# pollen-robotics/reachy2_symbolic_ik

Hardware: NVIDIA B200
Metric: ik_poses_per_sec (higher is better)
Workload: dtype f64

## Files before the change

### reachy2_symbolic_ik_b200/csrc/r2ik_device.cuh

```cuda
#pragma once

#include <math.h>
#include <stdint.h>

#include "../../include/r2ik.h"
#include "r2ik_math.cuh"

namespace r2ik {

constexpr double kPi = 3.14159265358979323846;
constexpr double kTwoPi = 2.0 * kPi;
constexpr double kHalfPi = kPi / 2;

struct ArmConst {
  double s[3];
  double L1, L2, L12;
  double L1sq, L2sq;
  double wo[3];
  double to[3];
  double tip_z;
  double max_arm_length;
  double d_min;
  double proj_margin;
  double backward_limit;
  double nvm;
  double rL, rLsq, hL;
  double Mst[9];
  double Pst[3];
  double es[3];
  double sing_coeff, sing_offset;
  double plP[3], plV[3];
  double plC[3], plRho;
  double elbow_limit;
  double side;
};



template <bool LIT>
R2IK_HD void cs_of_atan2(double y, double x, double &c, double &s, bool &degenerate) {
  if (LIT) {
    sincos(atan2(y, x), &s, &c);
  } else {
    double h2 = x * x + y * y;
    degenerate = degenerate || !((unsigned)(hi_word(h2) - 0x05e00000) < (unsigned)(0x7a000000 - 0x05e00000));
    double ih = rsqrt_pos(h2);
    c = x * ih; s = y * ih;
  }
}

template <bool LIT>
R2IK_HD double cs_and_angle(double y, double x, double &c, double &s, bool &degenerate) {
  cs_of_atan2<LIT>(y, x, c, s, degenerate);
  if (LIT) return atan2(y, x);
  return angle_of_unit(c, s);
}

template <bool LIT>
R2IK_HD double atan2_leaf(double y, double x, bool &degenerate) {
  if (LIT) return atan2(y, x);
  degenerate = degenerate || !atan2_core_ok(y, x);
  return atan2_core(y, x);
}

#if defined(__CUDACC__)
__device__ __noinline__ double2 sincos_library_dev(double a) {
  double s, c;
  sincos(a, &s, &c);
  return make_double2(s, c);
}
#endif
R2IK_HD void sincos_any(double a, double &s, double &c) {
  if (sincos_small_ok(a)) { sincos_small(a, s, c); return; }
#if defined(__CUDA_ARCH__)
  double2 r = sincos_library_dev(a);
  s = r.x; c = r.y;
#else
  sincos(a, &s, &c);
#endif
}

R2IK_HD double pymod(double a, double m) {
  double r = fmod(a, m);
  if (r != 0.0) {
    if ((m < 0.0) != (r < 0.0)) r += m;
  } else {
    r = copysign(0.0, m);
  }
  return r;
}

R2IK_HD double pymod_2pi_not_minus_zero(double x) {
  const double two_pi = R2IK_WRAP(1), four_pi = R2IK_WRAP(2);
  if (!(x >= -two_pi && x < R2IK_WRAP(3))) return pymod(x, kTwoPi);
  double r = x >= four_pi ? x - four_pi : x;
  r = r >= two_pi ? r - two_pi : r;
  return x < 0.0 ? x + two_pi : r;
}
R2IK_HD double pymod_2pi(double x) { return pymod_2pi_not_minus_zero(x) + 0.0; }

R2IK_HD double angle_diff(double a, double b) { return pymod_2pi_not_minus_zero((a - b) + R2IK_WRAP(0)) - R2IK_WRAP(0); }

R2IK_HD bool np_isclose(double a, double b) { return fabs(a - b) <= 1e-8 + 1e-5 * fabs(b); }

R2IK_HD bool is_valid_angle(double angle, double i0, double i1) {
  if (pymod_2pi(i0) == pymod_2pi(i1)) return true;
  if (i0 < i1) return (i0 <= angle) && (angle <= i1);
  return (i0 <= angle) || (angle <= i1);
}

R2IK_HD double limit_theta_to_interval(double theta, double i0, double i1) {
  theta = pymod_2pi(theta);
  if (theta > kPi) theta -= kTwoPi;
  if (is_valid_angle(theta, i0, i1)) return theta;
  double pos_diff = angle_diff(theta, i1);
  double neg_diff = angle_diff(theta, i0);
  if (fabs(pos_diff) < fabs(neg_diff)) return i1;
  return i0;
}

R2IK_HD double mul_add_unfused(double a, double b, double c) {
#if defined(__CUDA_ARCH__)
  return __dadd_rn(__dmul_rn(a, b), c);
#else
  return a * b + c;
#endif
}

struct Linspace {
  double start, stop, delta, step;
  int div;
};
R2IK_HD Linspace make_linspace(double start, double stop, int num) {
  Linspace L;
  L.start = start; L.stop = stop; L.div = num - 1; L.delta = stop - start;
  L.step = L.div > 0 ? L.delta / (double)L.div : 0.0;
  return L;
}
R2IK_HD double linspace_value(const Linspace &L, int i) {
  if (L.div <= 0) return L.start;
  if (i == L.div) return L.stop;
  if (L.step == 0.0) return mul_add_unfused((double)i / (double)L.div, L.delta, L.start);
  return mul_add_unfused((double)i, L.step, L.start);
}

R2IK_HD void search_range(double i0, double i1, double &start, double &stop) {
  if (fabs(fabs(i0) + fabs(i1) - kTwoPi) < 0.00001) { start = kHalfPi; stop = kHalfPi + kTwoPi; }
  else if (i0 < i1) { start = i0; stop = i1; }
  else { start = i0; stop = i1 + kTwoPi; }
}

struct Quat { double x, y, z, w; };

R2IK_HD Quat quat_mul(const Quat &p, const Quat &q) {
  Quat o;
  o.x = p.w * q.x + q.w * p.x + (p.y * q.z - p.z * q.y);
  o.y = p.w * q.y + q.w * p.y + (p.z * q.x - p.x * q.z);
  o.z = p.w * q.z + q.w * p.z + (p.x * q.y - p.y * q.x);
  o.w = p.w * q.w - p.x * q.x - p.y * q.y - p.z * q.z;
  return o;
}

R2IK_HD Quat quat_axis(int axis, double angle) {
  double s, c;
  sincos(angle / 2.0, &s, &c);
  Quat q = {0.0, 0.0, 0.0, c};
  if (axis == 0) q.x = s; else if (axis == 1) q.y = s; else q.z = s;
  return q;
}

R2IK_HD Quat quat_from_euler(int a0, int a1, int a2, bool intrinsic, double e0, double e1, double e2) {
  Quat q = quat_axis(a0, e0);
  Quat q1 = quat_axis(a1, e1);
  q = intrinsic ? quat_mul(q, q1) : quat_mul(q1, q);
  Quat q2 = quat_axis(a2, e2);
  q = intrinsic ? quat_mul(q, q2) : quat_mul(q2, q);
  return q;
}

R2IK_HD void quat_to_matrix(const Quat &q, double m[9]) {
  double x2 = q.x * q.x, y2 = q.y * q.y, z2 = q.z * q.z, w2 = q.w * q.w;
  double xy = q.x * q.y, zw = q.z * q.w, xz = q.x * q.z, yw = q.y * q.w, yz = q.y * q.z, xw = q.x * q.w;
  m[0] = x2 - y2 - z2 + w2; m[1] = 2 * (xy - zw);       m[2] = 2 * (xz + yw);
  m[3] = 2 * (xy + zw);     m[4] = -x2 + y2 - z2 + w2;  m[5] = 2 * (yz - xw);
  m[6] = 2 * (xz - yw);     m[7] = 2 * (yz + xw);       m[8] = -x2 - y2 + z2 + w2;
}

R2IK_HD void rot_from_euler_xyz(double e0, double e1, double e2, double m[9]) {
  double sx, cx, sy, cy, sz, cz;
  sincos_any(e0 / 2.0, sx, cx);
  sincos_any(e1 / 2.0, sy, cy);
  sincos_any(e2 / 2.0, sz, cz);
  Quat a = {cy * sx, cx * sy, -(sy * sx), cy * cx};
  Quat q;
  q.x = cz * a.x - sz * a.y;
  q.y = cz * a.y + sz * a.x;
  q.z = cz * a.z + a.w * sz;
  q.w = cz * a.w - sz * a.z;
  quat_to_matrix(q, m);
}

R2IK_HD double det3(const double m[9]) {
  return m[0] * (m[4] * m[8] - m[5] * m[7]) - m[1] * (m[3] * m[8] - m[5] * m[6]) + m[2] * (m[3] * m[7] - m[4] * m[6]);
}

R2IK_HD void polar_orthogonalize(double m[9]) {
  double mx = 0.0;
  for (int k = 0; k < 9; ++k) mx = fmax(mx, fabs(m[k]));
  if (mx < 0.0625 || (mx > 16.0 && mx < INFINITY)) {
    const int e = ilogb(mx);
    for (int k = 0; k < 9; ++k) m[k] = ldexp(m[k], -e);
  }
  bool last = false;
  for (int it = 0; it < 60; ++it) {
    double id = 1.0 / det3(m);
    double c[9];
    c[0] = (m[4] * m[8] - m[5] * m[7]) * id; c[1] = (m[5] * m[6] - m[3] * m[8]) * id; c[2] = (m[3] * m[7] - m[4] * m[6]) * id;
    c[3] = (m[2] * m[7] - m[1] * m[8]) * id; c[4] = (m[0] * m[8] - m[2] * m[6]) * id; c[5] = (m[1] * m[6] - m[0] * m[7]) * id;
    c[6] = (m[1] * m[5] - m[2] * m[4]) * id; c[7] = (m[2] * m[3] - m[0] * m[5]) * id; c[8] = (m[0] * m[4] - m[1] * m[3]) * id;
    double delta = 0.0;
    for (int k = 0; k < 9; ++k) {
      double nx = 0.5 * (m[k] + c[k]);
      delta = fmax(delta, fabs(nx - m[k]));
      m[k] = nx;
    }
    if (last) break;
    if (delta < 1e-8) last = true;
  }
}

R2IK_HD bool quat_from_matrix(const double min[9], Quat &q) {
  double m[9];
  for (int k = 0; k < 9; ++k) m[k] = min[k];
  if (!(det3(m) > 0.0)) return false;
  bool orthogonal = true;
  for (int i = 0; i < 3; ++i)
    for (int j = i; j < 3; ++j) {
      double g = m[3 * i] * m[3 * j] + m[3 * i + 1] * m[3 * j + 1] + m[3 * i + 2] * m[3 * j + 2];
      double e = (i == j) ? 1.0 : 0.0;
      if (!(fabs(g - e) <= 1e-12 + 1e-5 * e)) orthogonal = false;
    }
  if (!orthogonal) polar_orthogonalize(m);
  double tr = m[0] + m[4] + m[8];
  int choice = 0;
  double best = m[0];
  if (m[4] > best) { best = m[4]; choice = 1; }
  if (m[8] > best) { best = m[8]; choice = 2; }
  if (tr > best) { choice = 3; }
  if (choice == 0) {
    q.x = 1 - tr + 2 * m[0]; q.y = m[3] + m[1]; q.z = m[6] + m[2]; q.w = m[7] - m[5];
  } else if (choice == 1) {
    q.x = m[3] + m[1]; q.y = 1 - tr + 2 * m[4]; q.z = m[7] + m[5]; q.w = m[2] - m[6];
  } else if (choice == 2) {
    q.x = m[6] + m[2]; q.y = m[7] + m[5]; q.z = 1 - tr + 2 * m[8]; q.w = m[3] - m[1];
  } else {
    q.x = m[7] - m[5]; q.y = m[2] - m[6]; q.z = m[3] - m[1]; q.w = 1 + tr;
  }
  double n = sqrt(q.x * q.x + q.y * q.y + q.z * q.z + q.w * q.w);
  q.x /= n; q.y /= n; q.z /= n; q.w /= n;
  return true;
}

R2IK_HD void get_angles(bool extrinsic, bool symmetric, double sign, double a, double b, double c, double d, double out[3]) {
  const double eps = 1e-7;
  double half_sum = atan2(b, a);
  double half_diff = atan2(d, c);
  double ang0 = 0.0, ang2 = 0.0;
  double ang1 = 2 * atan2(hypot(c, d), hypot(a, b));
  bool case1 = fabs(ang1) <= eps;
  bool case2 = fabs(ang1 - kPi) <= eps;
  bool case0 = !(case1 || case2);
  ang0 = case1 ? 2 * half_sum : 2 * half_diff * (extrinsic ? -1.0 : 1.0);
  double first, third;
  if (extrinsic) {
    first = case0 ? half_sum - half_diff : ang0;
    third = case0 ? half_sum + half_diff : ang2;
  } else {
    first = case0 ? half_sum - half_diff : ang2;
    third = case0 ? half_sum + half_diff : ang0;
  }
  if (!symmetric) {
    third = third * sign;
    ang1 = ang1 - kHalfPi;
  }
  if (extrinsic) { ang0 = first; ang2 = third; } else { ang2 = first; ang0 = third; }
  out[0] = pymod_2pi(ang0 + kPi) - kPi;
  out[1] = pymod_2pi(ang1 + kPi) - kPi;
  out[2] = pymod_2pi(ang2 + kPi) - kPi;
}

R2IK_HD void quat_as_euler_xyz_extrinsic(const Quat &q, double out[3]) {
  get_angles(true, false, 1.0, q.w - q.y, q.x + q.z, q.y + q.w, q.z - q.x, out);
}
R2IK_HD void quat_as_euler_XYZ_intrinsic(const Quat &q, double out[3]) {
  get_angles(false, false, -1.0, q.w - q.y, q.z - q.x, q.y + q.w, -q.x - q.z, out);
}
R2IK_HD void quat_as_euler_ZYZ_intrinsic(const Quat &q, double out[3]) {
  get_angles(false, true, -1.0, q.w, q.z, q.y, q.x * -1.0, out);
}

R2IK_HD bool euler_xyz_from_mat4(const double *M, double e[3]) {
  double m9[9] = {M[0], M[1], M[2], M[4], M[5], M[6], M[8], M[9], M[10]};
  Quat q;
  if (!quat_from_matrix(m9, q)) return false;
  quat_as_euler_xyz_extrinsic(q, e);
  return true;
}

R2IK_HD bool rotation_is_identity(const double *M) {
  bool close = true;
  for (int i = 0; i < 3; ++i)
    for (int j = 0; j < 3; ++j) {
      double e = (i == j) ? 1.0 : 0.0;
      if (!(fabs(M[4 * i + j] - e) <= 1e-8 + 1e-5 * e)) close = false;
    }
  return close;
}

R2IK_HD void limit_orbita3d_wrist(double j[7], double max_angle) {
  {
    const double a = j[4], b = j[5], c = j[6];
    if (fabs(a) <= kPi && fabs(c) <= kPi && fabs(b) < kHalfPi - 1e-3 && sincos_small_ok(max_angle)) {
      if (a == 0.0 && b == 0.0) return;
      double sa, ca, sb, cb, sm, cm;
      sincos_small(a, sa, ca);
      sincos_small(b, sb, cb);
      sincos_small(max_angle, sm, cm);
      const double cbeta = ca * cb;
      if (cbeta < 1.0 - 1e-12) {
        if (cbeta >= cm) return;
        double sc, cc;
        sincos_small(c, sc, cc);
        const double r02 = sb, r12 = -sa * cb;
        const double r20 = sa * sc - ca * sb * cc, r21 = sa * cc + ca * sb * sc;
        const double isb = rsqrt_pos(r02 * r02 + r12 * r12);
        const double cal = r02 * isb, sal = r12 * isb, cga = -r20 * isb, sga = r21 * isb;
        const double q02 = cal * sm, q12 = sal * sm, q22 = cm;
        const double q00 = cal * cm * cga - sal * sga, q01 = -(cal * cm) * sga - sal * cga;
        j[4] = atan2_core(-q12, q22);
        j[5] = atan2_core(q02, sqrt_nonneg(q12 * q12 + q22 * q22));
        j[6] = atan2_core(-q01, q00);
        return;
      }
    }
  }
  Quat q = quat_from_euler(0, 1, 2, true, j[4], j[5], j[6]);
  double zyz[3];
  quat_as_euler_ZYZ_intrinsic(q, zyz);
  zyz[1] = fmin(max_angle, fmax(-max_angle, zyz[1]));
  Quat q2 = quat_from_euler(2, 1, 2, true, zyz[0], zyz[1], zyz[2]);
  double rpy[3];
  quat_as_euler_XYZ_intrinsic(q2, rpy);
  j[4] = rpy[0]; j[5] = rpy[1]; j[6] = rpy[2];
}

struct Solve {
  double p[3];
  double R[9];
  double w[3];
  double c[3];
  double r;
  double a1[3];
  double a2[3];
};

R2IK_HD void rmfv_columns(double vx, double vy, double vz, bool normalise, double c0[3], double a1[3], double a2[3]) {
  double ux = vx, uy = vy, uz = vz;
  if (normalise) {
    double in = rsqrt_pos(vx * vx + vy * vy + vz * vz);
    ux = vx * in; uy = vy * in; uz = vz * in;
  }
  if (np_isclose(1.0, ux) && np_isclose(0.0, uy) && np_isclose(0.0, uz)) {
    c0[0] = 1; c0[1] = 0; c0[2] = 0;
    a1[0] = 0; a1[1] = 1; a1[2] = 0;
    a2[0] = 0; a2[1] = 0; a2[2] = 1;
    return;
  }
  if (np_isclose(1.0, -ux) && np_isclose(0.0, -uy) && np_isclose(0.0, -uz)) {
    c0[0] = -1; c0[1] = 0; c0[2] = 0;
    a1[0] = 0; a1[1] = 1; a1[2] = 0;
    a2[0] = 0; a2[1] = 0; a2[2] = -1;
    return;
  }
  double f = div_fast(1.0 - ux, uy * uy + uz * uz);
  c0[0] = 1.0 + (-(uy * uy) - (uz * uz)) * f; c0[1] = uy; c0[2] = uz;
  a1[0] = -uy; a1[1] = 1.0 + (-(uy * uy)) * f; a1[2] = (-(uy * uz)) * f;
  a2[0] = -uz; a2[1] = (-(uy * uz)) * f;       a2[2] = 1.0 + (-(uz * uz)) * f;
}

R2IK_HD void wrist_from_goal(const ArmConst &A, const double p[3], const double R[9], double w[3]) {
  w[0] = R[0] * A.wo[0] + R[1] * A.wo[1] + R[2] * A.wo[2] + p[0];
  w[1] = R[3] * A.wo[0] + R[4] * A.wo[1] + R[5] * A.wo[2] + p[1];
  w[2] = R[6] * A.wo[0] + R[7] * A.wo[1] + R[8] * A.wo[2] + p[2];
}

R2IK_HD void reduce_goal(const ArmConst &A, double p[3], double w[3], double d, double d_target) {
  double sc = div_fast(d_target, fabs(d) + A.proj_margin);
  for (int k = 0; k < 3; ++k) {
    double nw = A.s[k] + (w[k] - A.s[k]) * sc;
    p[k] = p[k] + (nw - w[k]);
    w[k] = nw;
  }
}

template <bool WANT_R>
R2IK_HD bool elbow_circle(const ArmConst &A, Solve &S, double d, double invd, double n[3], double &r2) {
  double Px = S.w[0] - A.s[0], Py = S.w[1] - A.s[1], Pz = S.w[2] - A.s[2];
  if (d > A.L12) return false;
  double d2 = d * d;
  double k = d2 - A.L2sq + A.L1sq;
  double inv2d = 0.5 * invd;
  double rad = 4.0 * d2 * A.L1sq - k * k;
  r2 = rad * (inv2d * inv2d);
  if (WANT_R) S.r = hi_word(rad) < 0 ? NAN : inv2d * sqrt_nonneg(rad);
  double cd = k * inv2d;
  n[0] = Px * invd; n[1] = Py * invd; n[2] = Pz * invd;
  S.c[0] = n[0] * cd + A.s[0];
  S.c[1] = n[1] * cd + A.s[1];
  S.c[2] = n[2] * cd + A.s[2];
  return true;
}

struct Reach {
  int state;
  double i0, i1;
  double c0, s0;
  bool degenerate;
  bool literal;
};

constexpr double kSinMinusPi = -1.2246467991473532e-16;

R2IK_HD int reach_prechecks(const ArmConst &A, double &px, double &py, double &pz) {
  int pre_state = -1;
  double dx = px - A.s[0], dy = py - A.s[1], dz = pz - A.s[2];
  const double dg2 = dx * dx + dy * dy + dz * dz, L2 = A.max_arm_length * A.max_arm_length;
  bool outside = dg2 > L2;
  if (fabs(dg2 - L2) <= 1e-12) outside = sqrt(dg2) > A.max_arm_length;
  if (outside) {
    double sc = dg2 < INFINITY ? div_fast(A.max_arm_length, sqrt_nonneg(dg2) + A.proj_margin) : 0.0;
    px = A.s[0] + dx * sc;
    py = A.s[1] + dy * sc;
    pz = A.s[2] + dz * sc;
    pre_state = R2IK_STATE_POSE_OUT_OF_REACH;
  }
  if (px < A.backward_limit) {
    px = A.backward_limit;
    pre_state = R2IK_STATE_BACKWARD_POSE;
  }
  return pre_state;
}

template <bool NO_LIMITS, bool FLAG_ONLY, bool LIT, bool CIRCLE_ONLY = false>
R2IK_HD Reach solve_core_impl(const ArmConst &A, Solve &S) {
  Reach out;
  out.i0 = NAN; out.i1 = NAN; out.c0 = NAN; out.s0 = NAN; out.degenerate = false; out.literal = false;
  wrist_from_goal(A, S.p, S.R, S.w);
  if (S.w[0] < A.backward_limit) {
    double diff = A.backward_limit - S.w[0];
    S.p[0] = S.p[0] + diff;
    if (NO_LIMITS) wrist_from_goal(A, S.p, S.R, S.w);
    else S.w[0] = S.w[0] + diff;
  }
  double d, invd;
  {
    double dx = S.w[0] - A.s[0], dy = S.w[1] - A.s[1], dz = S.w[2] - A.s[2];
    d = sqrt_rsqrt_nonneg(dx * dx + dy * dy + dz * dz, invd);
  }
  bool moved = false;
  if (d > A.L12) {
    if (!NO_LIMITS) { out.state = R2IK_STATE_WRIST_OUT_OF_RANGE; return out; }
    reduce_goal(A, S.p, S.w, d, A.L12);
    moved = true;
  }
  if (d < A.d_min) {
    reduce_goal(A, S.p, S.w, d, A.d_min);
    wrist_from_goal(A, S.p, S.R, S.w);
    moved = true;
  }
  if (moved) {
    double dx = S.w[0] - A.s[0], dy = S.w[1] - A.s[1], dz = S.w[2] - A.s[2];
    d = sqrt_rsqrt_nonneg(dx * dx + dy * dy + dz * dz, invd);
  }
  double n[3], r2;
  if (!elbow_circle<!FLAG_ONLY || LIT>(A, S, d, invd, n, r2)) { out.state = R2IK_STATE_SHOULD_NOT_HAPPEN; return out; }
  if (!FLAG_ONLY) {
    double c0[3];
    rmfv_columns(n[0], n[1], n[2], false, c0, S.a1, S.a2);
  }
  if (NO_LIMITS) {
    out.state = R2IK_STATE_REACHABLE; out.i0 = -kPi; out.i1 = kPi; out.c0 = -1.0; out.s0 = kSinMinusPi;
    return out;
  }
  if (CIRCLE_ONLY) { out.state = R2IK_STATE_REACHABLE; return out; }

  double nLx = S.w[0] - S.p[0], nLy = S.w[1] - S.p[1], nLz = S.w[2] - S.p[2];
  double inLn = rsqrt_pos(nLx * nLx + nLy * nLy + nLz * nLz);
  double n1[3] = {nLx * inLn, nLy * inLn, nLz * inLn};
  double p1[3] = {n1[0] * A.hL, n1[1] * A.hL, n1[2] * A.hL};
  double p2[3] = {S.c[0] - S.w[0], S.c[1] - S.w[1], S.c[2] - S.w[2]};
  const double *n2 = n;
  if (!LIT) {
    const double b0 = p2[0] - p1[0], b1 = p2[1] - p1[1], b2 = p2[2] - p1[2];
    const double Xc = n1[0] * b0 + n1[1] * b1 + n1[2] * b2;
    const double nb = n2[0] * b0 + n2[1] * b1 + n2[2] * b2;
    double Aa = 0.0, Ba = 0.0, rho2;
    if (FLAG_ONLY) {
      const double Ca = n1[0] * n2[0] + n1[1] * n2[1] + n1[2] * n2[2];
      rho2 = fma(-Ca, Ca, 1.0);
    } else {
      Aa = n1[0] * S.a1[0] + n1[1] * S.a1[1] + n1[2] * S.a1[2];
      Ba = n1[0] * S.a2[0] + n1[1] * S.a2[1] + n1[2] * S.a2[2];
      rho2 = Aa * Aa + Ba * Ba;
    }
    const double rr = r2 * rho2;
    const double dl = rr - Xc * Xc;
    bool deg = fabs(n1[1]) < 1e-7 && fabs(n1[2]) < 1e-7;
    deg = deg || !(rho2 > 1e-12);
    deg = deg || fabs(Xc - nb) <= 1e-8 + 1e-5 * fabs(nb);
    deg = deg || !(r2 > 0.0) || fabs(dl) <= 1e-12 * (rr + Xc * Xc);
    out.degenerate = out.degenerate || deg;
    if (dl < 0.0) {
      if (Xc > 0) { out.state = R2IK_STATE_REACHABLE; out.i0 = -kPi; out.i1 = kPi; out.c0 = -1.0; out.s0 = kSinMinusPi; }
      else out.state = R2IK_STATE_LIMITED_BY_WRIST;
      return out;
    }
    out.state = R2IK_STATE_REACHABLE;
    if (FLAG_ONLY) return out;
    const double irr = rsqrt_pos(rr);
    const double kappa = -Xc * irr, sp = sqrt_nonneg(dl) * irr;
    const double irho = rsqrt_pos(rho2);
    const double cph = Aa * irho, sph = Ba * irho;
    const double c_lo = cph * kappa + sph * sp, s_lo = sph * kappa - cph * sp;
    const double c_hi = cph * kappa - sph * sp, s_hi = sph * kappa + cph * sp;
    out.i0 = angle_of_unit(c_lo, s_lo);
    out.i1 = angle_of_unit(c_hi, s_hi);
    out.c0 = c_lo; out.s0 = s_lo;
    return out;
  }
  double l0[3], t1[3], t2[3];
  rmfv_columns(n1[0], n1[1], n1[2], false, l0, t1, t2);
  double Xc = l0[0] * (p2[0] - p1[0]) + l0[1] * (p2[1] - p1[1]) + l0[2] * (p2[2] - p1[2]);

  bool linked_full = false, decided = false;
  {
    bool pa = (fabs(n2[0] - n1[0]) < A.nvm) && (fabs(n2[1] - n1[1]) < A.nvm) && (fabs(n2[2] - n1[2]) < A.nvm);
    bool pb = (fabs(n2[0] + n1[0]) < A.nvm) && (fabs(n2[1] + n1[1]) < A.nvm) && (fabs(n2[2] + n1[2]) < A.nvm);
    if (pa || pb) { decided = true; linked_full = Xc > 0; }
  }
  double q[3], v[3];
  if (!decided) {
    v[0] = n1[1] * n2[2] - n1[2] * n2[1];
    v[1] = n1[2] * n2[0] - n1[0] * n2[2];
    v[2] = n1[0] * n2[1] - n1[1] * n2[0];
    double inv = rsqrt_pos(v[0] * v[0] + v[1] * v[1] + v[2] * v[2]);
    v[0] *= inv; v[1] *= inv; v[2] *= inv;
    double e1[3] = {v[1] * n1[2] - v[2] * n1[1], v[2] * n1[0] - v[0] * n1[2], v[0] * n1[1] - v[1] * n1[0]};
    double b[3] = {p2[0] - p1[0], p2[1] - p1[1], p2[2] - p1[2]};
    double t = (n2[0] * b[0] + n2[1] * b[1] + n2[2] * b[2]) * inv;
    double u = (n1[0] * b[0] + n1[1] * b[1] + n1[2] * b[2]) * inv;
    if (np_isclose(u, t)) { decided = true; linked_full = Xc > 0; }
    q[0] = e1[0] * t + p1[0]; q[1] = e1[1] * t + p1[1]; q[2] = e1[2] * t + p1[2];
  }
  if (!decided) {
    double wv[3] = {q[0] - p1[0], q[1] - p1[1], q[2] - p1[2]};
    double qa = v[0] * v[0] + v[1] * v[1] + v[2] * v[2];
    double qb = 2.0 * (v[0] * wv[0] + v[1] * wv[1] + v[2] * wv[2]);
    double qc = (wv[0] * wv[0] + wv[1] * wv[1] + wv[2] * wv[2]) - A.rLsq;
    double disc = qb * qb - 4.0 * qa * qc;
    if (disc < 0) {
      decided = true; linked_full = Xc > 0;
    } else if (FLAG_ONLY) {
      out.state = R2IK_STATE_REACHABLE;
      return out;
    } else {
      double sq = sqrt_nonneg(disc);
      double inv2a = rcp_fast(2.0 * qa);
      double ta = (disc == 0) ? (-qb * inv2a) : ((-qb + sq) * inv2a);
      double Pa[3] = {q[0] + ta * v[0] - p2[0], q[1] + ta * v[1] - p2[1], q[2] + ta * v[2] - p2[2]};
      double ya = S.a2[0] * Pa[0] + S.a2[1] * Pa[1] + S.a2[2] * Pa[2];
      double xa = S.a1[0] * Pa[0] + S.a1[1] * Pa[1] + S.a1[2] * Pa[2];
      double ca, sa;
      double ang1 = cs_and_angle<LIT>(ya, xa, ca, sa, out.degenerate);
      if (disc == 0) {
        out.state = R2IK_STATE_REACHABLE; out.i0 = ang1; out.i1 = ang1;
        out.c0 = ca; out.s0 = sa;
        return out;
      }
      double tb = (-qb - sq) * inv2a;
      double Pb[3] = {q[0] + tb * v[0] - p2[0], q[1] + tb * v[1] - p2[1], q[2] + tb * v[2] - p2[2]};
      double yb = S.a2[0] * Pb[0] + S.a2[1] * Pb[1] + S.a2[2] * Pb[2];
      double xb = S.a1[0] * Pb[0] + S.a1[1] * Pb[1] + S.a1[2] * Pb[2];
      double cb, sb;
      double ang2 = cs_and_angle<LIT>(yb, xb, cb, sb, out.degenerate);
      if (ang2 < ang1) {
        double tmp = ang1; ang1 = ang2; ang2 = tmp;
        tmp = ca; ca = cb; cb = tmp;
        tmp = sa; sa = sb; sb = tmp;
      }
      double sm, cm;
      if (LIT) {
        sincos((ang1 + ang2) / 2.0, &sm, &cm);
      } else {
        double bx = ca + cb, by = sa + sb;
        double b2 = bx * bx + by * by;
        out.degenerate = out.degenerate || !(b2 > 1e-12);
        double ib = rsqrt_pos(b2);
        if (ang2 - ang1 > kPi) ib = -ib;
        cm = bx * ib; sm = by * ib;
      }
      double yc = cm * S.r, zc = sm * S.r;
      double Tm[3] = {S.a1[0] * yc + S.a2[0] * zc + p2[0] - p1[0], S.a1[1] * yc + S.a2[1] * zc + p2[1] - p1[1],
                      S.a1[2] * yc + S.a2[2] * zc + p2[2] - p1[2]};
      double xl = l0[0] * Tm[0] + l0[1] * Tm[1] + l0[2] * Tm[2];
      out.state = R2IK_STATE_REACHABLE;
      if (xl > 0) { out.i0 = ang1; out.i1 = ang2; out.c0 = ca; out.s0 = sa; }
      else { out.i0 = ang2; out.i1 = ang1; out.c0 = cb; out.s0 = sb; }
      return out;
    }
  }
  if (linked_full) { out.state = R2IK_STATE_REACHABLE; out.i0 = -kPi; out.i1 = kPi; out.c0 = -1.0; out.s0 = kSinMinusPi; }
  else out.state = R2IK_STATE_LIMITED_BY_WRIST;
  return out;
}

template <bool NO_LIMITS, bool FLAG_ONLY>
#if defined(__CUDACC__)
__host__ __device__ __noinline__
#else
inline
#endif
void solve_core_literal(const ArmConst &A, Solve *S, Reach *out) {
  *out = solve_core_impl<NO_LIMITS, FLAG_ONLY, true>(A, *S);
}

template <bool NO_LIMITS, bool FLAG_ONLY>
R2IK_HD Reach solve_core(const ArmConst &A, Solve &S) {
  const double p0 = S.p[0], p1 = S.p[1], p2 = S.p[2];
  Reach out = solve_core_impl<NO_LIMITS, FLAG_ONLY, false>(A, S);
  if (out.degenerate) {
    Solve T;
    T.p[0] = p0; T.p[1] = p1; T.p[2] = p2;
    for (int k = 0; k < 9; ++k) T.R[k] = S.R[k];
    Reach lit;
    solve_core_literal<NO_LIMITS, FLAG_ONLY>(A, &T, &lit);
    S = T;
    out = lit;
    out.literal = true;
  }
  return out;
}

R2IK_HD void circle_of_reachable(const ArmConst &A, const double pos[3], Solve &S) {
  S.p[0] = pos[0]; S.p[1] = pos[1]; S.p[2] = pos[2];
  solve_core_impl<false, false, false, true>(A, S);
}

template <bool NO_LIMITS>
R2IK_HD Reach is_reachable_R(const ArmConst &A, const double pos[3], Solve &S) {
  double px = pos[0], py = pos[1], pz = pos[2];
  int pre_state = reach_prechecks(A, px, py, pz);
  if (!NO_LIMITS && pre_state >= 0) {
    Reach out;
    out.state = pre_state; out.i0 = NAN; out.i1 = NAN; out.c0 = NAN; out.s0 = NAN; out.degenerate = false; out.literal = false;
    return out;
  }
  S.p[0] = px; S.p[1] = py; S.p[2] = pz;
  return solve_core<NO_LIMITS, false>(A, S);
}

template <bool NO_LIMITS>
R2IK_HD Reach is_reachable(const ArmConst &A, const double pos[3], const double eul[3], Solve &S) {
  rot_from_euler_xyz(eul[0], eul[1], eul[2], S.R);
  return is_reachable_R<NO_LIMITS>(A, pos, S);
}

R2IK_HD void elbow_position_cs(const Solve &S, double ct, double st, double E[3]) {
  double y = S.r * ct, z = S.r * st;
  E[0] = S.a1[0] * y + S.a2[0] * z + S.c[0];
  E[1] = S.a1[1] * y + S.a2[1] * z + S.c[1];
  E[2] = S.a1[2] * y + S.a2[2] * z + S.c[2];
}

R2IK_HD void elbow_position(const Solve &S, double theta, double E[3]) {
  double st, ct;
  sincos_any(theta, st, ct);
  double y = S.r * ct, z = S.r * st;
  E[0] = S.a1[0] * y + S.a2[0] * z + S.c[0];
  E[1] = S.a1[1] * y + S.a2[1] * z + S.c[1];
  E[2] = S.a1[2] * y + S.a2[2] * z + S.c[2];
}

R2IK_HD bool is_elbow_ok(const ArmConst &A, const double E[3]) {
  bool ok = (E[1] * A.side < -0.2);
  ok = ok && (E[2] < (E[0] - A.es[0]) * A.sing_coeff + A.es[2] - A.sing_offset);
  return ok;
}

R2IK_HD bool elbow_projection_fires(const ArmConst &A, const double E[3]) {
  return E[2] > (E[0] - A.es[0]) * A.sing_coeff + A.es[2] - A.sing_offset;
}

struct P3 { double x, y, z; };
R2IK_HD void rot_y(P3 &p, double c, double s) {
  double x = c * p.x + s * p.z, z = -s * p.x + c * p.z;
  p.x = x; p.z = z;
}
R2IK_HD void rot_z(P3 &p, double c, double s) {
  double x = c * p.x - s * p.y, y = s * p.x + c * p.y;
  p.x = x; p.y = y;
}
R2IK_HD void rot_x(P3 &p, double c, double s) {
  double y = c * p.y - s * p.z, z = s * p.y + c * p.z;
  p.y = y; p.z = z;
}
R2IK_HD P3 to_shoulder(const ArmConst &A, const double X[3]) {
  P3 o;
  o.x = A.Mst[0] * X[0] + A.Mst[1] * X[1] + A.Mst[2] * X[2] + A.Pst[0];
  o.y = A.Mst[3] * X[0] + A.Mst[4] * X[1] + A.Mst[5] * X[2] + A.Pst[1];
  o.z = A.Mst[6] * X[0] + A.Mst[7] * X[1] + A.Mst[8] * X[2] + A.Pst[2];
  return o;
}

template <bool LIT>
R2IK_HD bool get_joints_impl(const ArmConst &A, Solve &S, double ct, double st, double prev0, double prev2, double joints[7],
                             double E[3]) {
  bool degenerate = false;
  elbow_position_cs(S, ct, st, E);
  if (elbow_projection_fires(A, E)) {
    double dist = (E[0] - A.plP[0]) * A.plV[0] + (E[1] - A.plP[1]) * A.plV[1] + (E[2] - A.plP[2]) * A.plV[2];
    double vc[3] = {E[0] - dist * A.plV[0] - A.plC[0], E[1] - dist * A.plV[1] - A.plC[1], E[2] - dist * A.plV[2] - A.plC[2]};
    double sc = A.plRho * rsqrt_pos(vc[0] * vc[0] + vc[1] * vc[1] + vc[2] * vc[2]);
    for (int k = 0; k < 3; ++k) {
      double ne = A.plC[k] + vc[k] * sc;
      S.p[k] = S.p[k] + (ne - E[k]);
      E[k] = ne;
    }
    wrist_from_goal(A, S.p, S.R, S.w);
  }
  double tipw[3] = {S.R[0] * A.to[0] + S.R[1] * A.to[1] + S.R[2] * A.to[2] + S.p[0],
                    S.R[3] * A.to[0] + S.R[4] * A.to[1] + S.R[5] * A.to[2] + S.p[1],
                    S.R[6] * A.to[0] + S.R[7] * A.to[1] + S.R[8] * A.to[2] + S.p[2]};
  double ptw[3] = {S.R[0] * 0.1 + tipw[0], S.R[3] * 0.1 + tipw[1], S.R[6] * 0.1 + tipw[2]};
  P3 el = to_shoulder(A, E), wr = to_shoulder(A, S.w), tp = to_shoulder(A, tipw), pt = to_shoulder(A, ptw);
  double s, c;

  double at[7];
  const bool sing0 = is_zero(el.x) && is_zero(el.z);
  if (LIT && sing0) { at[0] = 0.0; sincos(-prev0, &s, &c); }
  else at[0] = cs_and_angle<LIT>(el.z, el.x, c, s, degenerate);
  rot_y(el, c, s); rot_y(wr, c, s); rot_y(tp, c, s); rot_y(pt, c, s);
  at[1] = -cs_and_angle<LIT>(-el.y, el.x, c, s, degenerate);
  rot_z(wr, c, s); rot_z(tp, c, s); rot_z(pt, c, s);
  wr.x -= A.L1; tp.x -= A.L1; pt.x -= A.L1;
  const bool sing2 = is_zero(wr.y) && is_zero(wr.z);
  if (LIT && sing2) { at[2] = 0.0; sincos(prev2, &s, &c); }
  else {
    double ca, sa;
    at[2] = cs_and_angle<LIT>(wr.z, -wr.y, ca, sa, degenerate);
    c = sa; s = -ca;
  }
  rot_x(wr, c, s); rot_x(tp, c, s); rot_x(pt, c, s);
  at[3] = cs_and_angle<LIT>(wr.z, wr.x, c, s, degenerate);
  rot_y(tp, c, s); rot_y(pt, c, s);
  tp.x -= A.L2; pt.x -= A.L2;
  {
    double ca, sa;
    at[4] = cs_and_angle<LIT>(tp.y, -tp.x, ca, sa, degenerate);
    c = -ca; s = -sa;
  }
  rot_z(tp, c, s); rot_z(pt, c, s);
  at[5] = cs_and_angle<LIT>(tp.z, tp.x, c, s, degenerate);
  rot_y(pt, c, s);
  at[6] = atan2_leaf<LIT>(pt.y, pt.z, degenerate);
  double shoulder_pitch = sing0 ? prev0 : -at[0];
  double shoulder_roll = at[1];
  double elbow_yaw = sing2 ? prev2 : -kHalfPi + at[2];
  double elbow_pitch = -at[3];
  double wrist_roll = kPi - at[4];
  if (wrist_roll > kPi) wrist_roll = wrist_roll - kTwoPi;
  double wrist_pitch = at[5];
  double wrist_yaw = -at[6];

  joints[0] = shoulder_pitch; joints[1] = shoulder_roll; joints[2] = elbow_yaw; joints[3] = elbow_pitch;
  joints[4] = wrist_roll; joints[5] = -wrist_pitch; joints[6] = -wrist_yaw;
  if (joints[3] > A.elbow_limit) joints[3] = A.elbow_limit;
  if (joints[3] < -A.elbow_limit) joints[3] = -A.elbow_limit;
  return !degenerate;
}

#if defined(__CUDACC__)
__host__ __device__ __noinline__
#else
inline
#endif
void get_joints_literal(const ArmConst &A, Solve *S, double ct, double st, double prev0, double prev2, double *joints,
                        double *E) {
  get_joints_impl<true>(A, *S, ct, st, prev0, prev2, joints, E);
}

R2IK_HD void get_joints_cs(const ArmConst &A, Solve &S, double ct, double st, double prev0, double prev2, double joints[7],
                           double E[3]) {
  const double p0 = S.p[0], p1 = S.p[1], p2 = S.p[2], w0 = S.w[0], w1 = S.w[1], w2 = S.w[2];
  if (!get_joints_impl<false>(A, S, ct, st, prev0, prev2, joints, E)) {
    Solve T = S;
    T.p[0] = p0; T.p[1] = p1; T.p[2] = p2; T.w[0] = w0; T.w[1] = w1; T.w[2] = w2;
    double jj[7], EE[3];
    get_joints_literal(A, &T, ct, st, prev0, prev2, jj, EE);
    S = T;
    for (int k = 0; k < 7; ++k) joints[k] = jj[k];
    for (int k = 0; k < 3; ++k) E[k] = EE[k];
  }
}

R2IK_HD void get_joints(const ArmConst &A, Solve &S, double theta, double prev0, double prev2, double joints[7], double E[3]) {
  double st, ct;
  sincos_any(theta, st, ct);
  get_joints_cs(A, S, ct, st, prev0, prev2, joints, E);
}

R2IK_HD bool pose_from_mat4(const double *M, bool snap, double pos[3], double eul[3]) {
  pos[0] = M[3]; pos[1] = M[7]; pos[2] = M[11];
  if (snap && rotation_is_identity(M)) { eul[0] = 0.0; eul[1] = 0.0; eul[2] = 0.0; return true; }
  return euler_xyz_from_mat4(M, eul);
}

#if defined(__CUDACC__)
__host__ __device__ __noinline__
#else
inline
#endif
bool rotation_from_mat3_literal(const double m[9], double R[9]) {
  if (!(det3(m) > 0.0)) return false;
  {
    bool orthogonal = true;
    for (int i = 0; i < 3; ++i)
      for (int j = i; j < 3; ++j) {
        double g = m[3 * i] * m[3 * j] + m[3 * i + 1] * m[3 * j + 1] + m[3 * i + 2] * m[3 * j + 2];
        double e = (i == j) ? 1.0 : 0.0;
        if (!(fabs(g - e) <= 1e-12 + 1e-5 * e)) orthogonal = false;
      }
    if (!orthogonal) {
      double p[9];
      for (int k = 0; k < 9; ++k) p[k] = m[k];
      polar_orthogonalize(p);
      if (p[0] * p[0] + p[3] * p[3] > 1e-10) {
        for (int k = 0; k < 9; ++k) R[k] = p[k];
        return true;
      }
    }
  }
  double e[3];
  Quat q;
  if (!quat_from_matrix(m, q)) return false;
  quat_as_euler_xyz_extrinsic(q, e);
  rot_from_euler_xyz(e[0], e[1], e[2], R);
  return true;
}

R2IK_HD bool rotation_from_mat4(const double *M, bool snap, double R[9]) {
  if (snap && rotation_is_identity(M)) {
    R[0] = 1; R[1] = 0; R[2] = 0; R[3] = 0; R[4] = 1; R[5] = 0; R[6] = 0; R[7] = 0; R[8] = 1;
    return true;
  }
  const double m[9] = {M[0], M[1], M[2], M[4], M[5], M[6], M[8], M[9], M[10]};
  bool direct = true;
  for (int i = 0; i < 3; ++i)
    for (int j = i; j < 3; ++j) {
      double g = m[3 * i] * m[3 * j] + m[3 * i + 1] * m[3 * j + 1] + m[3 * i + 2] * m[3 * j + 2];
      double e = (i == j) ? 1.0 : 0.0;
      if (!(fabs(g - e) <= 1e-13)) direct = false;
    }
  if (!(m[0] * m[0] + m[3] * m[3] > 1e-10)) direct = false;
  if (!(det3(m) > 0.0)) direct = false;
  if (direct) {
    for (int k = 0; k < 9; ++k) R[k] = m[k];
    return true;
  }
  double mm[9], RR[9];
  for (int k = 0; k < 9; ++k) mm[k] = m[k];
  bool ok = rotation_from_mat3_literal(mm, RR);
  for (int k = 0; k < 9; ++k) R[k] = RR[k];
  return ok;
}

R2IK_HD constexpr int pose_stride(int kind) { return kind == R2IK_POSE_EULER6 ? 6 : kind == R2IK_POSE_MAT34 ? 12 : 16; }

R2IK_HD void load2(const double *p, double &a, double &b) {
#if defined(__CUDA_ARCH__)
  const double2 v = __ldg(reinterpret_cast<const double2 *>(p));
  a = v.x; b = v.y;
#else
  a = p[0]; b = p[1];
#endif
}

R2IK_HD void load_mat4(const double *M, double m[16]) {
#pragma unroll
  for (int r = 0; r < 3; ++r) {
    load2(M + 4 * r, m[4 * r], m[4 * r + 1]);
    load2(M + 4 * r + 2, m[4 * r + 2], m[4 * r + 3]);
  }
  m[12] = 0.0; m[13] = 0.0; m[14] = 0.0; m[15] = 1.0;
}

template <int KIND>
R2IK_HD bool load_pose(const double *row, bool snap, double pos[3], double R[9]) {
  if (KIND == R2IK_POSE_EULER6) {
    double e[3];
    load2(row, pos[0], pos[1]);
    load2(row + 2, pos[2], e[0]);
    load2(row + 4, e[1], e[2]);
    rot_from_euler_xyz(e[0], e[1], e[2], R);
    return true;
  }
  double m[16];
  load_mat4(row, m);
  pos[0] = m[3]; pos[1] = m[7]; pos[2] = m[11];
  return rotation_from_mat4(m, snap, R);
}

template <int KIND, bool NO_LIMITS = false>
R2IK_HD Reach symik_reach(const ArmConst &A, const double *row, Solve &S) {
  double pos[3];
  Reach rc;
  rc.state = R2IK_STATE_INVALID_ROTATION; rc.i0 = NAN; rc.i1 = NAN;
  if (load_pose<KIND>(row, false, pos, S.R)) rc = is_reachable_R<NO_LIMITS>(A, pos, S);
  return rc;
}

R2IK_HD void symik_joints(const ArmConst &A, Solve &S, const Reach &rc, const double *theta, double prev0, double prev2,
                          double j[7], double E[3]) {
  if (rc.state == R2IK_STATE_REACHABLE) {
    double ct = rc.c0, st = rc.s0;
    if (theta) sincos_any(*theta, st, ct);
    get_joints_cs(A, S, ct, st, prev0, prev2, j, E);
  } else {
#pragma unroll
    for (int k = 0; k < 7; ++k) j[k] = NAN;
    E[0] = NAN; E[1] = NAN; E[2] = NAN;
  }
}

template <int KIND>
R2IK_HD bool symik_no_limits(const ArmConst &A, const double *row, const double *theta, const double *prev, double j[7],
                             double E[3]) {
  double pos[3];
  Solve S;
  bool ok = load_pose<KIND>(row, false, pos, S.R);
  if (ok) ok = is_reachable_R<true>(A, pos, S).state == R2IK_STATE_REACHABLE;
  bool proj = false;
  if (ok) {
    double prev0 = 0.0, prev2 = 0.0;
    if (prev) { prev0 = prev[0]; prev2 = prev[2]; }
    double st, ct, Ep[3];
    sincos_any(*theta, st, ct);
    elbow_position_cs(S, ct, st, Ep);
    proj = elbow_projection_fires(A, Ep);
    get_joints_cs(A, S, ct, st, prev0, prev2, j, E);
  } else {
    for (int k = 0; k < 7; ++k) j[k] = NAN;
    E[0] = NAN; E[1] = NAN; E[2] = NAN;
  }
  return proj;
}

template <int KIND, bool NO_LIMITS>
R2IK_HD bool pose_elbow_circle(const ArmConst &A, const double *row, Solve &S) {
  double pos[3];
  bool ok = load_pose<KIND>(row, false, pos, S.R);
  if (ok) {
    const int st = is_reachable_R<NO_LIMITS>(A, pos, S).state;
    ok = st == R2IK_STATE_REACHABLE || (!NO_LIMITS && st == R2IK_STATE_LIMITED_BY_WRIST);
  }
  return ok;
}

R2IK_HD double sweep_theta(const Reach &rc, const double *row, int K, int k) {
  if (rc.state != R2IK_STATE_REACHABLE) return NAN;
  if (row) return row[k];
  double start, stop;
  search_range(rc.i0, rc.i1, start, stop);
  return linspace_value(make_linspace(start, stop, K), k);
}

R2IK_HD bool sweep_sample(const ArmConst &A, const Solve &S0, const Reach &rc, double theta, double prev0, double prev2,
                          double j[7], double E[3]) {
  if (rc.state != R2IK_STATE_REACHABLE) {
    for (int k = 0; k < 7; ++k) j[k] = NAN;
    E[0] = NAN; E[1] = NAN; E[2] = NAN;
    return false;
  }
  Solve S = S0;
  double st, ct, Ep[3];
  sincos_any(theta, st, ct);
  elbow_position_cs(S, ct, st, Ep);
  const bool proj = elbow_projection_fires(A, Ep);
  get_joints_cs(A, S, ct, st, prev0, prev2, j, E);
  return proj;
}

R2IK_HD bool elbow_on_circle(const ArmConst &A, const Solve &S, bool circle, const double *theta, double E[3]) {
  E[0] = NAN; E[1] = NAN; E[2] = NAN;
  if (!circle) return false;
  double st, ct;
  sincos_any(*theta, st, ct);
  elbow_position_cs(S, ct, st, E);
  return elbow_projection_fires(A, E);
}

}
```

Measured before the change: 15.36 billion.

## Simplify fast-path joint extraction by exploiting rotation structure and direction vectors

```diff
diff --git a/reachy2_symbolic_ik_b200/csrc/r2ik_device.cuh b/reachy2_symbolic_ik_b200/csrc/r2ik_device.cuh
--- a/reachy2_symbolic_ik_b200/csrc/r2ik_device.cuh
+++ b/reachy2_symbolic_ik_b200/csrc/r2ik_device.cuh
@@ -37,14 +37,17 @@
 
 
 
+R2IK_HD double rsqrt_norm2(double h2, bool &degenerate) {
+  degenerate = degenerate || !((unsigned)(hi_word(h2) - 0x05e00000) < (unsigned)(0x7a000000 - 0x05e00000));
+  return rsqrt_pos(h2);
+}
+
 template <bool LIT>
 R2IK_HD void cs_of_atan2(double y, double x, double &c, double &s, bool &degenerate) {
   if (LIT) {
     sincos(atan2(y, x), &s, &c);
   } else {
-    double h2 = x * x + y * y;
-    degenerate = degenerate || !((unsigned)(hi_word(h2) - 0x05e00000) < (unsigned)(0x7a000000 - 0x05e00000));
-    double ih = rsqrt_pos(h2);
+    double ih = rsqrt_norm2(x * x + y * y, degenerate);
     c = x * ih; s = y * ih;
   }
 }
@@ -738,41 +741,77 @@
     }
     wrist_from_goal(A, S.p, S.R, S.w);
   }
-  double tipw[3] = {S.R[0] * A.to[0] + S.R[1] * A.to[1] + S.R[2] * A.to[2] + S.p[0],
-                    S.R[3] * A.to[0] + S.R[4] * A.to[1] + S.R[5] * A.to[2] + S.p[1],
-                    S.R[6] * A.to[0] + S.R[7] * A.to[1] + S.R[8] * A.to[2] + S.p[2]};
-  double ptw[3] = {S.R[0] * 0.1 + tipw[0], S.R[3] * 0.1 + tipw[1], S.R[6] * 0.1 + tipw[2]};
-  P3 el = to_shoulder(A, E), wr = to_shoulder(A, S.w), tp = to_shoulder(A, tipw), pt = to_shoulder(A, ptw);
-  double s, c;
+  P3 el = to_shoulder(A, E), wr = to_shoulder(A, S.w);
 
   double at[7];
-  const bool sing0 = is_zero(el.x) && is_zero(el.z);
-  if (LIT && sing0) { at[0] = 0.0; sincos(-prev0, &s, &c); }
-  else at[0] = cs_and_angle<LIT>(el.z, el.x, c, s, degenerate);
-  rot_y(el, c, s); rot_y(wr, c, s); rot_y(tp, c, s); rot_y(pt, c, s);
-  at[1] = -cs_and_angle<LIT>(-el.y, el.x, c, s, degenerate);
-  rot_z(wr, c, s); rot_z(tp, c, s); rot_z(pt, c, s);
-  wr.x -= A.L1; tp.x -= A.L1; pt.x -= A.L1;
-  const bool sing2 = is_zero(wr.y) && is_zero(wr.z);
-  if (LIT && sing2) { at[2] = 0.0; sincos(prev2, &s, &c); }
-  else {
-    double ca, sa;
-    at[2] = cs_and_angle<LIT>(wr.z, -wr.y, ca, sa, degenerate);
-    c = sa; s = -ca;
-  }
-  rot_x(wr, c, s); rot_x(tp, c, s); rot_x(pt, c, s);
-  at[3] = cs_and_angle<LIT>(wr.z, wr.x, c, s, degenerate);
-  rot_y(tp, c, s); rot_y(pt, c, s);
-  tp.x -= A.L2; pt.x -= A.L2;
-  {
-    double ca, sa;
-    at[4] = cs_and_angle<LIT>(tp.y, -tp.x, ca, sa, degenerate);
-    c = -ca; s = -sa;
-  }
-  rot_z(tp, c, s); rot_z(pt, c, s);
-  at[5] = cs_and_angle<LIT>(tp.z, tp.x, c, s, degenerate);
-  rot_y(pt, c, s);
-  at[6] = atan2_leaf<LIT>(pt.y, pt.z, degenerate);
+  bool sing0 = false, sing2 = false;
+  if constexpr (LIT) {
+    double tipw[3] = {S.R[0] * A.to[0] + S.R[1] * A.to[1] + S.R[2] * A.to[2] + S.p[0],
+                      S.R[3] * A.to[0] + S.R[4] * A.to[1] + S.R[5] * A.to[2] + S.p[1],
+                      S.R[6] * A.to[0] + S.R[7] * A.to[1] + S.R[8] * A.to[2] + S.p[2]};
+    double ptw[3] = {S.R[0] * 0.1 + tipw[0], S.R[3] * 0.1 + tipw[1], S.R[6] * 0.1 + tipw[2]};
+    P3 tp = to_shoulder(A, tipw), pt = to_shoulder(A, ptw);
+    double s, c;
+    sing0 = is_zero(el.x) && is_zero(el.z);
+    if (sing0) { at[0] = 0.0; sincos(-prev0, &s, &c); }
+    else at[0] = cs_and_angle<LIT>(el.z, el.x, c, s, degenerate);
+    rot_y(el, c, s); rot_y(wr, c, s); rot_y(tp, c, s); rot_y(pt, c, s);
+    at[1] = -cs_and_angle<LIT>(-el.y, el.x, c, s, degenerate);
+    rot_z(wr, c, s); rot_z(tp, c, s); rot_z(pt, c, s);
+    wr.x -= A.L1; tp.x -= A.L1; pt.x -= A.L1;
+    sing2 = is_zero(wr.y) && is_zero(wr.z);
+    if (sing2) { at[2] = 0.0; sincos(prev2, &s, &c); }
+    else {
+      double ca, sa;
+      at[2] = cs_and_angle<LIT>(wr.z, -wr.y, ca, sa, degenerate);
+      c = sa; s = -ca;
+    }
+    rot_x(wr, c, s); rot_x(tp, c, s); rot_x(pt, c, s);
+    at[3] = cs_and_angle<LIT>(wr.z, wr.x, c, s, degenerate);
+    rot_y(tp, c, s); rot_y(pt, c, s);
+    tp.x -= A.L2; pt.x -= A.L2;
+    {
+      double ca, sa;
+      at[4] = cs_and_angle<LIT>(tp.y, -tp.x, ca, sa, degenerate);
+      c = -ca; s = -sa;
+    }
+    rot_z(tp, c, s); rot_z(pt, c, s);
+    at[5] = cs_and_angle<LIT>(tp.z, tp.x, c, s, degenerate);
+    rot_y(pt, c, s);
+    at[6] = atan2_leaf<LIT>(pt.y, pt.z, degenerate);
+  } else {
+    const double h0 = el.x * el.x + el.z * el.z;
+    const double ir0 = rsqrt_norm2(h0, degenerate), in1 = rsqrt_norm2(h0 + el.y * el.y, degenerate);
+    const double c0 = el.x * ir0, s0 = el.z * ir0;
+    const double c1 = h0 * ir0 * in1, s1 = -el.y * in1;
+    at[0] = angle_of_unit(c0, s0);
+    at[1] = -angle_of_unit(c1, s1);
+    rot_y(wr, c0, s0); rot_z(wr, c1, s1); wr.x -= A.L1;
+    const double h2 = wr.y * wr.y + wr.z * wr.z;
+    const double n2 = h2 + wr.x * wr.x;
+    const double ir2 = rsqrt_norm2(h2, degenerate), in3 = rsqrt_norm2(n2, degenerate);
+    const double ca2 = -wr.y * ir2, sa2 = wr.z * ir2;
+    const double c2 = sa2, s2 = -ca2;
+    const double c3 = wr.x * in3, s3 = h2 * ir2 * in3;
+    at[2] = angle_of_unit(ca2, sa2);
+    at[3] = angle_of_unit(c3, s3);
+    P3 tz = {-A.tip_z * S.R[2], -A.tip_z * S.R[5], -A.tip_z * S.R[8]}, ux = {S.R[0], S.R[3], S.R[6]};
+    P3 tp = {A.Mst[0] * tz.x + A.Mst[1] * tz.y + A.Mst[2] * tz.z, A.Mst[3] * tz.x + A.Mst[4] * tz.y + A.Mst[5] * tz.z,
+             A.Mst[6] * tz.x + A.Mst[7] * tz.y + A.Mst[8] * tz.z};
+    P3 pt = {A.Mst[0] * ux.x + A.Mst[1] * ux.y + A.Mst[2] * ux.z, A.Mst[3] * ux.x + A.Mst[4] * ux.y + A.Mst[5] * ux.z,
+             A.Mst[6] * ux.x + A.Mst[7] * ux.y + A.Mst[8] * ux.z};
+    rot_y(tp, c0, s0); rot_z(tp, c1, s1); rot_x(tp, c2, s2); rot_y(tp, c3, s3);
+    tp.x += n2 * in3 - A.L2;
+    const double h4 = tp.x * tp.x + tp.y * tp.y;
+    const double ir4 = rsqrt_norm2(h4, degenerate), in5 = rsqrt_norm2(h4 + tp.z * tp.z, degenerate);
+    const double ca4 = -tp.x * ir4, sa4 = tp.y * ir4;
+    const double c5 = h4 * ir4 * in5, s5 = tp.z * in5;
+    at[4] = angle_of_unit(ca4, sa4);
+    at[5] = angle_of_unit(c5, s5);
+    rot_y(pt, c0, s0); rot_z(pt, c1, s1); rot_x(pt, c2, s2); rot_y(pt, c3, s3);
+    rot_z(pt, -ca4, -sa4); rot_y(pt, c5, s5);
+    at[6] = atan2_leaf<LIT>(pt.y, pt.z, degenerate);
+  }
   double shoulder_pitch = sing0 ? prev0 : -at[0];
   double shoulder_roll = at[1];
   double elbow_yaw = sing2 ? prev2 : -kHalfPi + at[2];
```

Result: no change. 15.29 billion, median of 6 (-0.5%).
